# SHI-Labs/Self-Similarity-Grouping

Hardware: AMD Instinct MI355X
Metric: images/s embed + s/iter for NxN rerank+DBSCAN, N=16k, 1/2/4/8 GPU (higher is better)
Workload: dtype f32 (embed: split-half operands hi+lo on fp16 MFMA, fp32 accumulate, 6e-8 max error vs the fp32 reference features) / exact int64 via int8 MFMA digits + f64 + f16 (distance, re-rank: half semantics, bit-exact)

## Files before the change

self-similarity-grouping_amd/csrc/bottleneck.hip:

```cpp
#include "ssg_common.h"
#include <cstdlib>

#ifndef SSG_BN_NT_STORE
#define SSG_BN_NT_STORE 1
#endif
#ifndef SSG_BN_NT_RES
#define SSG_BN_NT_RES 1
#endif

namespace ssg {
namespace bneck {

typedef float v16f __attribute__((ext_vector_type(16)));
typedef unsigned int v4u __attribute__((ext_vector_type(4)));
typedef _Float16 v8h __attribute__((ext_vector_type(8)));
typedef float v4f __attribute__((ext_vector_type(4)));

struct Params {
  const float* x; float* out;
  const float* w1; const float* b1; const float* cs1;
  const float* w2; const float* b2; const float* cs2;
  const float* w3; const float* b3; const float* cs3;
  int B, H;
  int* overflow;
  unsigned long long* prof = nullptr;
};
#ifdef SSG_BN_PROF
#define SSG_BN_STAMP(I_) { if (p.prof && threadIdx.x == 0) p.prof[(size_t)blockIdx.x * 8 + (I_)] = __builtin_readcyclecounter(); }
#else
#define SSG_BN_STAMP(I_)
#endif

constexpr int cmax(int a, int b) { return a > b ? a : b; }

template <int C, int MID, int IW, int TH, int CIN = C, int NW = 4>
struct Cfg {
  static constexpr int HROWS = TH + 2, NPIX1 = HROWS * IW, NPIX = TH * IW;
  static constexpr int NTHR = NW * 64, RPP = NTHR / 4;
#ifndef SSG_BN_K1T
#define SSG_BN_K1T 32
#endif
#ifndef SSG_BN_K1T4
#define SSG_BN_K1T4 32
#endif
  static constexpr int K1T = NW == 8 ? SSG_BN_K1T : SSG_BN_K1T4, KS1 = K1T / 16, CPR1 = 4 * KS1, RPP1 = NTHR / CPR1;
  static constexpr int XROWS = (NPIX1 + RPP1 - 1) / RPP1 * RPP1;
  static constexpr int P1 = 80;
  static constexpr int P1T = K1T * 4 + 16;
  static constexpr int KT2 = NW == 8 ? 2 : 1;
  static constexpr int P2 = KT2 * 128 + 16;
  static constexpr int PY = MID * 4 + 16;
  static constexpr int BUF1 = (XROWS + MID) * P1T;
  static constexpr int ZERO_OFF = NPIX1 * PY;
  static constexpr int W2_OFF = (ZERO_OFF + PY + 255) / 256 * 256, BUF2 = MID * P2;
  static constexpr int W3_OFF = (NPIX * PY + 255) / 256 * 256, BUF3 = C * P1;
  static constexpr int LDS = cmax(cmax(2 * BUF1, W2_OFF + 2 * BUF2), W3_OFF + 2 * BUF3);
  static constexpr int DS = CIN != C;
#ifdef SSG_BN_ABL_NK1
  static constexpr int NK1 = SSG_BN_ABL_NK1;
#else
  static constexpr int NK1 = CIN / K1T;
#endif
  static constexpr int NK2 = (MID / 32) * 9 / KT2, NK3 = (MID + (DS ? CIN : 0)) / 16;
  static constexpr int PD1MAX = K1T == 64 ? 2 : (K1T == 32 ? 4 : 8);
  static constexpr int PD1 = NK1 < PD1MAX ? NK1 : PD1MAX, PD2 = KT2 == 1 ? 6 : 3;
  static_assert(((MID / 32) * 9) % KT2 == 0 && NK2 % PD2 == 0, "phase-2 stages and ring");
  static_assert((NW == 4 || NW == 8) && NPIX == 128 && NPIX1 % 32 == 0 && MID % RPP == 0 && MID % RPP1 == 0 && C % RPP == 0 && MID % (NW * 8) == 0, "128 output pixels, whole staging passes");
  static constexpr bool ZERO_EARLY = 2 * BUF1 <= ZERO_OFF;
  static_assert(LDS <= (NW == 4 ? 80 : 160) * 1024, "4 waves: two workgroups per CU; 8 waves: one");
  static_assert(NW == 4 || NW * 32 * 36 * 4 <= 2 * BUF3, "8 waves: the epilogue patches take over the W3 stages");
};

__device__ __forceinline__ unsigned pack2(_Float16 a, _Float16 b) {
  return (unsigned)__builtin_bit_cast(unsigned short, a) | ((unsigned)__builtin_bit_cast(unsigned short, b) << 16);
}
__device__ __forceinline__ void encode4(const float4 v, uint2& hi, uint2& lo) {
  const _Float16 h0 = (_Float16)v.x, h1 = (_Float16)v.y, h2 = (_Float16)v.z, h3 = (_Float16)v.w;
  hi = make_uint2(pack2(h0, h1), pack2(h2, h3));
  lo = make_uint2(pack2((_Float16)(v.x - (float)h0), (_Float16)(v.y - (float)h1)), pack2((_Float16)(v.z - (float)h2), (_Float16)(v.w - (float)h3)));
}
__device__ __forceinline__ unsigned hi_nonfinite_bits(const uint2 hi) {
  return ((hi.x & 0x7c007c00u) + 0x04000400u) | ((hi.y & 0x7c007c00u) + 0x04000400u);
}
__device__ __forceinline__ float hlo(unsigned u) { return (float)__builtin_bit_cast(_Float16, (unsigned short)(u & 0xffffu)); }
__device__ __forceinline__ float hhi(unsigned u) { return (float)__builtin_bit_cast(_Float16, (unsigned short)(u >> 16)); }
__device__ __forceinline__ float4 decode4(const uint2 hi, const uint2 lo) {
  return make_float4(hlo(hi.x) + hlo(lo.x), hhi(hi.x) + hhi(lo.x), hlo(hi.y) + hlo(lo.y), hhi(hi.y) + hhi(lo.y));
}
__device__ __forceinline__ float4 relu4(float4 v) {
  return make_float4(v.x > 0.f ? v.x : 0.f, v.y > 0.f ? v.y : 0.f, v.z > 0.f ? v.z : 0.f, v.w > 0.f ? v.w : 0.f);
}

__device__ __forceinline__ void bn_dma16(const __amdgpu_buffer_rsrc_t r, unsigned lds_addr, unsigned voff, int soff) {
  __builtin_amdgcn_raw_ptr_buffer_load_lds(r, (__attribute__((address_space(3))) void*)(uintptr_t)lds_addr, 16, voff, soff, 0, 0);
}

template <int C, int MID, int IW, int TH, int CIN, int NW>
__global__ __launch_bounds__(NW * 64, NW == 4 ? 2 : 1) void bottleneck_kernel(Params p) {
  using K = Cfg<C, MID, IW, TH, CIN, NW>;
  constexpr bool DS = K::DS;
  extern __shared__ __attribute__((aligned(16))) unsigned char smem[];
  const int tid = (int)threadIdx.x, lane = tid & 63, wave = tid >> 6, l32 = lane & 31, h = lane >> 5;
  const int tiles_img = p.H / TH, ntiles = p.B * tiles_img;
  int T;
  {
    const int b = (int)blockIdx.x, q = ntiles / 8, r = ntiles % 8, x = b % 8, s = b / 8;
    T = (x < r ? x * (q + 1) : r * (q + 1) + (x - r) * q) + s;
  }
  const int img = T / tiles_img, ty0 = (T - img * tiles_img) * TH;
  SSG_BN_STAMP(0)
  if (K::ZERO_EARLY && tid < K::PY / 16) *reinterpret_cast<uint4*>(smem + K::ZERO_OFF + tid * 16) = make_uint4(0u, 0u, 0u, 0u);

  constexpr int RPP = K::RPP, RPP1 = K::RPP1, AU = K::XROWS / RPP1, WU = MID / RPP1;
  const int ck = tid & 3, r0 = tid >> 2;
  const int ck1 = tid % K::CPR1, r1 = tid / K::CPR1;
  const float* ximg = p.x + (int64_t)img * p.H * IW * CIN;
  const __amdgpu_buffer_rsrc_t xrsrc = __builtin_amdgcn_make_buffer_rsrc(const_cast<float*>(ximg), 0, (unsigned)(p.H * IW * CIN * 4), 0x00020000);
  constexpr int MT1 = K::NPIX1 / 32, NT1 = MID / 32;
  constexpr int WC1 = NT1 < NW / 2 ? NT1 : NW / 2, WR1 = NW / WC1, MTW1 = (MT1 + WR1 - 1) / WR1, NTW1 = NT1 / WC1;
  static_assert(NT1 % WC1 == 0 && (WR1 * MTW1) * 32 <= K::XROWS, "phase-1 tiles divide over the waves");
  const int i1b = (wave / WC1) * MTW1, j1b = (wave % WC1) * NTW1;
  v16f acc1[MTW1][NTW1];
#pragma unroll
  for (int i = 0; i < MTW1; i++)
#pragma unroll
    for (int j = 0; j < NTW1; j++)
#pragma unroll
      for (int r = 0; r < 16; r++) acc1[i][j][r] = 0.f;
  float4 cs1r[NTW1][4], b1r[NTW1][4];
#pragma unroll
  for (int j = 0; j < NTW1; j++)
#pragma unroll
    for (int q = 0; q < 4; q++) {
      cs1r[j][q] = *reinterpret_cast<const float4*>(p.cs1 + (j1b + j) * 32 + 8 * q + 4 * h); b1r[j][q] = *reinterpret_cast<const float4*>(p.b1 + (j1b + j) * 32 + 8 * q + 4 * h);
    }
#ifndef SSG_BN_P1DMA
#define SSG_BN_P1DMA 1
#endif
  if constexpr (NW == 8 && K::K1T == 32 && SSG_BN_P1DMA) {
    constexpr int NS = 4, XR = K::NPIX1, SROWS = XR + MID, STG = SROWS * 128, NBLK = SROWS / 8, TDMA = (NBLK + NW - 1) / NW;
    static_assert(K::NK1 % NS == 0 && NS * STG <= K::LDS && SROWS % 8 == 0 && XR % 8 == 0 && MTW1 == 3 && NTW1 == 1, "phase-1 DMA stages");
    const int wv = __builtin_amdgcn_readfirstlane(wave);
    const __amdgpu_buffer_rsrc_t wrsrc = __builtin_amdgcn_make_buffer_rsrc(const_cast<float*>(p.w1), 0, (unsigned)(MID * CIN * 4), 0x00020000);
    unsigned go[TDMA];
    int gblk[TDMA];
#pragma unroll
    for (int u = 0; u < TDMA; u++) {
      int blk = wv + NW * u;
      if (blk >= NBLK) blk = wv;
      gblk[u] = blk;
      const int r = blk * 8 + (lane >> 3), lc = (lane & 7) ^ ((r >> 1) & 7);
      if (blk < XR / 8) {
        const int pix = (ty0 - 1) * IW + r;
        go[u] = (pix >= 0 && pix < p.H * IW) ? (unsigned)((pix * CIN + lc * 4) * 4) : 0x80000000u;
      } else {
        go[u] = (unsigned)(((r - XR) * CIN + lc * 4) * 4);
      }
    }
#define SSG_BN_DMA1(T_, ST_)                                                                                         \
    { _Pragma("unroll") for (int u = 0; u < TDMA; u++)                                                               \
        bn_dma16(gblk[u] < XR / 8 ? xrsrc : wrsrc, (unsigned)(uintptr_t)(smem + (ST_) * STG + gblk[u] * 1024), go[u], (T_) * 128); }
    const int i1s = __builtin_amdgcn_readfirstlane(i1b);
    int xo[MTW1], xs[MTW1];
#pragma unroll
    for (int i = 0; i < MTW1; i++) { const int r = (i1s + i) * 32 + l32; xo[i] = r * 128; xs[i] = (r >> 1) & 7; }
    const int wr_ = XR + j1b * 32 + l32, wo = wr_ * 128, ws = (wr_ >> 1) & 7;
    v8h fxh[2][2][MTW1], fxl[2][2][MTW1], fwh[2][2], fwl[2][2];
#define SSG_BN_READS1(ST_, S_)                                                                                       \
    { const unsigned char* sb_ = smem + (ST_) * STG;                                                                 \
      _Pragma("unroll") for (int ks = 0; ks < 2; ks++) {                                                             \
        _Pragma("unroll") for (int i = 0; i < MTW1; i++) {                                        \
          fxh[S_][ks][i] = *reinterpret_cast<const v8h*>(sb_ + xo[i] + (((4 * ks + 2 * h) ^ xs[i]) * 16));           \
          fxl[S_][ks][i] = *reinterpret_cast<const v8h*>(sb_ + xo[i] + (((4 * ks + 2 * h + 1) ^ xs[i]) * 16)); }     \
        fwh[S_][ks] = *reinterpret_cast<const v8h*>(sb_ + wo + (((4 * ks + 2 * h) ^ ws) * 16));                       \
        fwl[S_][ks] = *reinterpret_cast<const v8h*>(sb_ + wo + (((4 * ks + 2 * h + 1) ^ ws) * 16)); } }
#define SSG_BN_MMAK(S_, KS_)                                                                                         \
    { _Pragma("unroll") for (int i = 0; i < MTW1; i++) acc1[i][0] = __builtin_amdgcn_mfma_f32_32x32x16_f16(fwh[S_][KS_], fxl[S_][KS_][i], acc1[i][0], 0, 0, 0); \
      _Pragma("unroll") for (int i = 0; i < MTW1; i++) acc1[i][0] = __builtin_amdgcn_mfma_f32_32x32x16_f16(fwl[S_][KS_], fxh[S_][KS_][i], acc1[i][0], 0, 0, 0); \
      _Pragma("unroll") for (int i = 0; i < MTW1; i++) acc1[i][0] = __builtin_amdgcn_mfma_f32_32x32x16_f16(fwh[S_][KS_], fxh[S_][KS_][i], acc1[i][0], 0, 0, 0); }
#define SSG_BN_STEPD(KT_, ST_, STN_, S_)                                                                             \
    { SSG_BN_MMAK(S_, 0)                                                                                             \
      __builtin_amdgcn_sched_barrier(0);                                                                             \
      asm volatile("s_waitcnt vmcnt(%0) lgkmcnt(0)\n\ts_barrier" ::"n"(TDMA * (NS - 2)) : "memory");                  \
      { const int tn_ = (KT_) + NS < K::NK1 ? (KT_) + NS : K::NK1 - 1;    \
        SSG_BN_DMA1(tn_, ST_) }                                                                                      \
      SSG_BN_READS1(STN_, 1 - (S_))                                                                                  \
      __builtin_amdgcn_sched_barrier(0);                                                                             \
      SSG_BN_MMAK(S_, 1) }
    SSG_BN_DMA1(0, 0) SSG_BN_DMA1(1, 1) SSG_BN_DMA1(2, 2) SSG_BN_DMA1(3, 3)
    asm volatile("s_waitcnt vmcnt(%0)\n\ts_barrier" ::"n"(TDMA * (NS - 1)) : "memory");
    SSG_BN_READS1(0, 0)
#pragma unroll 1
    for (int kt = 0; kt < K::NK1; kt += NS) {
      SSG_BN_STEPD(kt, 0, 1, 0) SSG_BN_STEPD(kt + 1, 1, 2, 1) SSG_BN_STEPD(kt + 2, 2, 3, 0) SSG_BN_STEPD(kt + 3, 3, 0, 1)
    }
    __syncthreads();
#undef SSG_BN_STEPD
#undef SSG_BN_MMAK
#undef SSG_BN_READS1
#undef SSG_BN_DMA1
  } else {
  unsigned aoff[AU];
#pragma unroll
  for (int u = 0; u < AU; u++) {
    const int hp = r1 + RPP1 * u, pix = (ty0 - 1) * IW + hp;
    aoff[u] = (hp < K::NPIX1 && pix >= 0 && pix < p.H * IW) ? (unsigned)((pix * CIN + ck1 * 4) * 4) : 0x80000000u;
  }
  const float* w1p = p.w1 + (int64_t)r1 * CIN + ck1 * 4;
  v4f sa[K::PD1][AU], sw[K::PD1][WU];
#define SSG_BN_LOAD1(T_, S_)                                                                                         \
  {                                                                                                                  \
    _Pragma("unroll") for (int u = 0; u < AU; u++) {                                                                  \
      const v4u raw = __builtin_amdgcn_raw_buffer_load_b128(xrsrc, aoff[u], (T_) * (K::K1T * 4), 0);                  \
      sa[S_][u] = __builtin_bit_cast(v4f, raw);                                                                     \
    }                                                                                                                 \
    _Pragma("unroll") for (int u = 0; u < WU; u++) sw[S_][u] = *reinterpret_cast<const v4f*>(w1p + (int64_t)(RPP1 * u) * CIN + (T_) * K::K1T); \
  }
#define SSG_BN_STORE1(BUF_, S_)                                                                                      \
  {                                                                                                                  \
    unsigned char* sb_ = smem + (BUF_) * K::BUF1;                                                                    \
    _Pragma("unroll") for (int u = 0; u < AU; u++) *reinterpret_cast<v4f*>(sb_ + (r1 + RPP1 * u) * K::P1T + ck1 * 16) = sa[S_][u]; \
    _Pragma("unroll") for (int u = 0; u < WU; u++) *reinterpret_cast<v4f*>(sb_ + (K::XROWS + r1 + RPP1 * u) * K::P1T + ck1 * 16) = sw[S_][u]; \
  }
#define SSG_BN_MMA1(BUF_)                                                                                            \
  {                                                                                                                  \
    const unsigned char* sb_ = smem + (BUF_) * K::BUF1;                                                              \
    _Pragma("unroll") for (int ks = 0; ks < K::KS1; ks++) {                                                          \
    v8h xh_[MTW1], xl_[MTW1], wh_[NTW1], wl_[NTW1];                                                                  \
    _Pragma("unroll") for (int i = 0; i < MTW1; i++) {                                                               \
      const unsigned char* q_ = sb_ + ((i1b + i) * 32 + l32) * K::P1T + ks * 64 + h * 32;                            \
      xh_[i] = *reinterpret_cast<const v8h*>(q_); xl_[i] = *reinterpret_cast<const v8h*>(q_ + 16); }                 \
    _Pragma("unroll") for (int j = 0; j < NTW1; j++) {                                                               \
      const unsigned char* q_ = sb_ + (K::XROWS + (j1b + j) * 32 + l32) * K::P1T + ks * 64 + h * 32;                 \
      wh_[j] = *reinterpret_cast<const v8h*>(q_); wl_[j] = *reinterpret_cast<const v8h*>(q_ + 16); }                 \
    _Pragma("unroll") for (int i = 0; i < MTW1; i++) _Pragma("unroll") for (int j = 0; j < NTW1; j++)                \
      acc1[i][j] = __builtin_amdgcn_mfma_f32_32x32x16_f16(wh_[j], xl_[i], acc1[i][j], 0, 0, 0);                      \
    _Pragma("unroll") for (int i = 0; i < MTW1; i++) _Pragma("unroll") for (int j = 0; j < NTW1; j++)                \
      acc1[i][j] = __builtin_amdgcn_mfma_f32_32x32x16_f16(wl_[j], xh_[i], acc1[i][j], 0, 0, 0);                      \
    _Pragma("unroll") for (int i = 0; i < MTW1; i++) _Pragma("unroll") for (int j = 0; j < NTW1; j++)                \
      acc1[i][j] = __builtin_amdgcn_mfma_f32_32x32x16_f16(wh_[j], xh_[i], acc1[i][j], 0, 0, 0);                      \
    }                                                                                                                \
  }
#define SSG_BN_STEP1(KT_, S_)                                                                                        \
  {                                                                                                                  \
    if ((KT_) + K::PD1 < K::NK1) SSG_BN_LOAD1((KT_) + K::PD1, S_)    \
    SSG_BN_MMA1((S_) & 1)                                                                                            \
    if ((KT_) + 1 < K::NK1) SSG_BN_STORE1(((S_) + 1) & 1, ((S_) + 1) % K::PD1)                                        \
    __syncthreads();                                                                                                 \
  }
  static_assert(K::NK1 % K::PD1 == 0 && K::PD1 <= 8, "phase-1 ring of PD1 register sets");
#define SSG_BN_LOAD1_IF(S_) if constexpr ((S_) < K::PD1) SSG_BN_LOAD1(S_, S_)
  SSG_BN_LOAD1_IF(0) SSG_BN_LOAD1_IF(1) SSG_BN_LOAD1_IF(2) SSG_BN_LOAD1_IF(3) SSG_BN_LOAD1_IF(4) SSG_BN_LOAD1_IF(5) SSG_BN_LOAD1_IF(6) SSG_BN_LOAD1_IF(7)
#undef SSG_BN_LOAD1_IF
  SSG_BN_STORE1(0, 0)
  __syncthreads();
#define SSG_BN_STEP1_IF(KT_, S_) if constexpr ((S_) < K::PD1) SSG_BN_STEP1(KT_, S_)
#pragma unroll
  for (int kt0 = 0; kt0 < K::NK1; kt0 += K::PD1) {
    SSG_BN_STEP1_IF(kt0, 0) SSG_BN_STEP1_IF(kt0 + 1, 1) SSG_BN_STEP1_IF(kt0 + 2, 2) SSG_BN_STEP1_IF(kt0 + 3, 3)
    SSG_BN_STEP1_IF(kt0 + 4, 4) SSG_BN_STEP1_IF(kt0 + 5, 5) SSG_BN_STEP1_IF(kt0 + 6, 6) SSG_BN_STEP1_IF(kt0 + 7, 7)
  }
#undef SSG_BN_STEP1_IF
#undef SSG_BN_STEP1
  }
  SSG_BN_STAMP(1)
#undef SSG_BN_LOAD1
#undef SSG_BN_STORE1
#undef SSG_BN_MMA1

  constexpr int CPR2 = 8 * K::KT2, RP8 = K::NTHR / CPR2, BU = MID / RP8;
  const int ck8 = tid % CPR2, r8 = tid / CPR2;
  const float* w2p = p.w2 + (int64_t)r8 * (9 * MID) + ck8 * 4;
  v4f sb2[K::PD2][BU];
#define SSG_BN_LOAD2(T_, S_)                                                                                         \
  { _Pragma("unroll") for (int u = 0; u < BU; u++) sb2[S_][u] = *reinterpret_cast<const v4f*>(w2p + (int64_t)(RP8 * u) * (9 * MID) + (T_) * (32 * K::KT2)); }
#define SSG_BN_STORE2(BUF_, S_)                                                                                      \
  { unsigned char* sb_ = smem + K::W2_OFF + (BUF_) * K::BUF2;                                                        \
    _Pragma("unroll") for (int u = 0; u < BU; u++) *reinterpret_cast<v4f*>(sb_ + (r8 + RP8 * u) * K::P2 + ck8 * 16) = sb2[S_][u]; }
#define SSG_BN_LOAD2_IF(S_) if constexpr ((S_) < K::PD2) SSG_BN_LOAD2(S_, S_)
  SSG_BN_LOAD2_IF(0) SSG_BN_LOAD2_IF(1) SSG_BN_LOAD2_IF(2) SSG_BN_LOAD2_IF(3) SSG_BN_LOAD2_IF(4) SSG_BN_LOAD2_IF(5)
#undef SSG_BN_LOAD2_IF

  unsigned ovf = 0u;
#pragma unroll
  for (int i = 0; i < MTW1; i++) {
    if (i1b + i >= MT1) continue;
    const int hp0 = (i1b + i) * 32;
    const int irow = ty0 - 1 + (hp0 + l32) / IW;
    const bool inside = irow >= 0 && irow < p.H;
#pragma unroll
    for (int j = 0; j < NTW1; j++)
#pragma unroll
      for (int q = 0; q < 4; q++) {
        const int ch = (j1b + j) * 32 + 8 * q + 4 * h;
        const float4 cs = cs1r[j][q], bi = b1r[j][q];
        float4 v = make_float4(acc1[i][j][4 * q] * cs.x + bi.x, acc1[i][j][4 * q + 1] * cs.y + bi.y, acc1[i][j][4 * q + 2] * cs.z + bi.z,
                               acc1[i][j][4 * q + 3] * cs.w + bi.w);
        v = relu4(v);
        if (!inside) v = make_float4(0.f, 0.f, 0.f, 0.f);
        uint2 hi, lo;
        encode4(v, hi, lo);
        ovf |= hi_nonfinite_bits(hi);
        unsigned char* d = smem + (hp0 + l32) * K::PY + (ch >> 3) * 32 + h * 8;
        *reinterpret_cast<uint2*>(d) = hi; *reinterpret_cast<uint2*>(d + 16) = lo;
      }
  }
  if (!K::ZERO_EARLY && tid < K::PY / 16) *reinterpret_cast<uint4*>(smem + K::ZERO_OFF + tid * 16) = make_uint4(0u, 0u, 0u, 0u);
  SSG_BN_STORE2(0, 0)
  __syncthreads();
  SSG_BN_STAMP(2)

  constexpr int WC2 = NW / 4, NT2 = MID / 32 / WC2;
  const int pt2 = wave / WC2, cb2 = (wave % WC2) * NT2;
  v16f acc2[NT2];
#pragma unroll
  for (int j = 0; j < NT2; j++)
#pragma unroll
    for (int r = 0; r < 16; r++) acc2[j][r] = 0.f;
  const int m2 = pt2 * 32 + l32, ty2 = m2 / IW, tx2 = m2 - ty2 * IW;
  float4 cs2r[NT2][4], b2r[NT2][4];
#pragma unroll
  for (int j = 0; j < NT2; j++)
#pragma unroll
    for (int q = 0; q < 4; q++) {
      cs2r[j][q] = *reinterpret_cast<const float4*>(p.cs2 + (cb2 + j) * 32 + 8 * q + 4 * h); b2r[j][q] = *reinterpret_cast<const float4*>(p.b2 + (cb2 + j) * 32 + 8 * q + 4 * h);
    }
#define SSG_BN_STEP2(KT_, S_, B_)                                                                                     \
  {                                                                                                                  \
    if ((KT_) + K::PD2 < K::NK2) SSG_BN_LOAD2((KT_) + K::PD2, S_)                                                     \
    _Pragma("unroll") for (int sub = 0; sub < K::KT2; sub++) {                                                       \
      const int kt_ = (KT_) * K::KT2 + sub;                                                                          \
      const int chunk = kt_ / 9, tap = kt_ - chunk * 9, r = tap / 3, s = tap - r * 3;                                \
      const int xin = tx2 + s - 1;                                                                                   \
      const int abase = (xin >= 0 && xin < IW) ? ((ty2 + r) * IW + xin) * K::PY : K::ZERO_OFF;                       \
      const unsigned char* wb = smem + K::W2_OFF + (B_) * K::BUF2 + (cb2 * 32 + l32) * K::P2 + sub * 128 + h * 32;     \
      v8h xh_[2], xl_[2], wh_[2][NT2], wl_[2][NT2];                                                                  \
      _Pragma("unroll") for (int ks = 0; ks < 2; ks++) {                                                             \
        const unsigned char* q_ = smem + abase + (chunk * 4 + ks * 2 + h) * 32;                                      \
        xh_[ks] = *reinterpret_cast<const v8h*>(q_); xl_[ks] = *reinterpret_cast<const v8h*>(q_ + 16);               \
        _Pragma("unroll") for (int j = 0; j < NT2; j++) {                                                            \
          wh_[ks][j] = *reinterpret_cast<const v8h*>(wb + j * 32 * K::P2 + ks * 64);                                 \
          wl_[ks][j] = *reinterpret_cast<const v8h*>(wb + j * 32 * K::P2 + ks * 64 + 16); }                          \
      }                                                                                                              \
      _Pragma("unroll") for (int ks = 0; ks < 2; ks++) {                                                             \
        _Pragma("unroll") for (int j = 0; j < NT2; j++) acc2[j] = __builtin_amdgcn_mfma_f32_32x32x16_f16(wh_[ks][j], xl_[ks], acc2[j], 0, 0, 0); \
        _Pragma("unroll") for (int j = 0; j < NT2; j++) acc2[j] = __builtin_amdgcn_mfma_f32_32x32x16_f16(wl_[ks][j], xh_[ks], acc2[j], 0, 0, 0); \
        _Pragma("unroll") for (int j = 0; j < NT2; j++) acc2[j] = __builtin_amdgcn_mfma_f32_32x32x16_f16(wh_[ks][j], xh_[ks], acc2[j], 0, 0, 0); \
      }                                                                                                              \
    }                                                                                                                \
    if ((KT_) + 1 < K::NK2) SSG_BN_STORE2((B_) ^ 1, ((S_) + 1) % K::PD2)                                              \
    __syncthreads();                                                                                                 \
  }
  static_assert(K::NK2 % 6 == 0 && 6 % K::PD2 == 0, "phase-2 ring");
#pragma unroll
  for (int kt0 = 0; kt0 < K::NK2; kt0 += 6) {
    SSG_BN_STEP2(kt0, 0 % K::PD2, 0) SSG_BN_STEP2(kt0 + 1, 1 % K::PD2, 1) SSG_BN_STEP2(kt0 + 2, 2 % K::PD2, 0)
    SSG_BN_STEP2(kt0 + 3, 3 % K::PD2, 1) SSG_BN_STEP2(kt0 + 4, 4 % K::PD2, 0) SSG_BN_STEP2(kt0 + 5, 5 % K::PD2, 1)
  }
#undef SSG_BN_STEP2
  SSG_BN_STAMP(3)
#undef SSG_BN_LOAD2
#undef SSG_BN_STORE2

  constexpr int CU3 = C / RPP;
  constexpr int K3 = MID + (DS ? CIN : 0);
  const float* w3p = p.w3 + (int64_t)r0 * K3 + ck * 4;
  v4f sc3[2][CU3];
#define SSG_BN_LOAD3(T_, S_)                                                                                         \
  { _Pragma("unroll") for (int u = 0; u < CU3; u++) sc3[S_][u] = *reinterpret_cast<const v4f*>(w3p + (int64_t)(RPP * u) * K3 + (T_) * 16); }
#define SSG_BN_STORE3(BUF_, S_)                                                                                      \
  { unsigned char* sb_ = smem + K::W3_OFF + (BUF_) * K::BUF3;                                                        \
    _Pragma("unroll") for (int u = 0; u < CU3; u++) *reinterpret_cast<v4f*>(sb_ + (r0 + RPP * u) * K::P1 + ck * 16) = sc3[S_][u]; }
  SSG_BN_LOAD3(0, 0)
  SSG_BN_LOAD3(1, 1)
  constexpr int WC3 = NW / 4, NT3 = C / 32 / WC3;
  const int pt3 = wave / WC3, cb3 = (wave % WC3) * NT3;
  const int64_t gpix0 = ((int64_t)img * p.H + ty0) * IW + pt3 * 32;
  constexpr int NXK = DS ? CIN / 16 : 1;
  v8h xrh[NXK], xrl[NXK];
  if constexpr (DS) {
    const float* xq = p.x + (gpix0 + l32) * CIN + h * 8;
#pragma unroll
    for (int t = 0; t < NXK; t++) { xrh[t] = *reinterpret_cast<const v8h*>(xq + t * 16); xrl[t] = *reinterpret_cast<const v8h*>(xq + t * 16 + 4); }
  }
  unsigned char* myrows = smem + (pt3 * 32) * K::PY;
#pragma unroll
  for (int j = 0; j < NT2; j++)
#pragma unroll
    for (int q = 0; q < 4; q++) {
      const int ch = (cb2 + j) * 32 + 8 * q + 4 * h;
      const float4 cs = cs2r[j][q], bi = b2r[j][q];
      float4 v = make_float4(acc2[j][4 * q] * cs.x + bi.x, acc2[j][4 * q + 1] * cs.y + bi.y, acc2[j][4 * q + 2] * cs.z + bi.z, acc2[j][4 * q + 3] * cs.w + bi.w);
      v = relu4(v);
      uint2 hi, lo;
      encode4(v, hi, lo);
      ovf |= hi_nonfinite_bits(hi);
      unsigned char* d = smem + (pt2 * 32 + l32) * K::PY + (ch >> 3) * 32 + h * 8;
      *reinterpret_cast<uint2*>(d) = hi; *reinterpret_cast<uint2*>(d + 16) = lo;
    }

  static_assert(K::NK3 % 2 == 0, "phase 3 takes its k-tiles in rounds of two buffers");
  v16f acc3[NT3];
#pragma unroll
  for (int j = 0; j < NT3; j++)
#pragma unroll
    for (int r = 0; r < 16; r++) acc3[j][r] = 0.f;
#define SSG_BN_MMA3K(BUF_, KT_)                                                                                      \
  {                                                                                                                  \
    v8h xh_, xl_;                                                                                                    \
    if constexpr (DS && (KT_) >= MID / 16) { xh_ = xrh[((KT_) - MID / 16) % NXK]; xl_ = xrl[((KT_) - MID / 16) % NXK]; } \
    else {                                                                                                           \
      const unsigned char* q_ = myrows + l32 * K::PY + (((KT_) % (MID / 16)) * 2 + h) * 32;                          \
      xh_ = *reinterpret_cast<const v8h*>(q_); xl_ = *reinterpret_cast<const v8h*>(q_ + 16);                         \
    }                                                                                                                \
    const unsigned char* wb_ = smem + K::W3_OFF + (BUF_) * K::BUF3 + (cb3 * 32 + l32) * K::P1 + h * 32;              \
    _Pragma("unroll") for (int jj = 0; jj < NT3; jj += 4) {                                                          \
      v8h wh_[4], wl_[4];                                                                                            \
      _Pragma("unroll") for (int j = 0; j < 4; j++) {                                                                \
        wh_[j] = *reinterpret_cast<const v8h*>(wb_ + (jj + j) * 32 * K::P1); wl_[j] = *reinterpret_cast<const v8h*>(wb_ + (jj + j) * 32 * K::P1 + 16); } \
      _Pragma("unroll") for (int j = 0; j < 4; j++) acc3[jj + j] = __builtin_amdgcn_mfma_f32_32x32x16_f16(wh_[j], xl_, acc3[jj + j], 0, 0, 0); \
      _Pragma("unroll") for (int j = 0; j < 4; j++) acc3[jj + j] = __builtin_amdgcn_mfma_f32_32x32x16_f16(wl_[j], xh_, acc3[jj + j], 0, 0, 0); \
      _Pragma("unroll") for (int j = 0; j < 4; j++) acc3[jj + j] = __builtin_amdgcn_mfma_f32_32x32x16_f16(wh_[j], xh_, acc3[jj + j], 0, 0, 0); \
    }                                                                                                                \
  }
  constexpr int EP = 36, CPR = 8, RPI = 8, ITS = 4;
  const int chunk = lane % CPR, prow = lane / CPR, odd = lane & 1;
  const float* __restrict__ resp = p.x + gpix0 * C;
  float* __restrict__ outp = p.out + gpix0 * C;
  float4 rr[2][ITS], b3r[2], cs3r[2];
#ifdef SSG_BN_ABL_NORES
#define SSG_BN_RESLOAD(P_) make_float4(0.f, 0.f, 0.f, 0.f)
#elif SSG_BN_NT_RES
#define SSG_BN_RESLOAD(P_) ([&]() { const v4f t_ = __builtin_nontemporal_load(reinterpret_cast<const v4f*>(P_)); return make_float4(t_[0], t_[1], t_[2], t_[3]); }())
#else
#define SSG_BN_RESLOAD(P_) (*reinterpret_cast<const float4*>(P_))
#endif
  SSG_BN_STORE3(0, 0)
  SSG_BN_STORE3(1, 1)
  if constexpr (K::NK3 > 2) { SSG_BN_LOAD3(2, 0) SSG_BN_LOAD3(3, 1) }
  __syncthreads();
  static_assert(K::NK3 / 2 <= 4, "at most four rounds");
#define SSG_BN_ROUND3(R_)                                                                                            \
  if constexpr ((R_) < K::NK3 / 2) {                                                                                 \
    SSG_BN_MMA3K(0, 2 * (R_))                                                                                        \
    SSG_BN_MMA3K(1, 2 * (R_) + 1)                                                                                    \
    if constexpr ((R_) + 1 < K::NK3 / 2) {                                                                           \
      __syncthreads();                                                \
      SSG_BN_STORE3(0, 0)                                                                                            \
      SSG_BN_STORE3(1, 1)                                                                                            \
      if constexpr ((R_) + 2 < K::NK3 / 2) { SSG_BN_LOAD3(2 * (R_) + 4, 0) SSG_BN_LOAD3(2 * (R_) + 5, 1) }           \
      else {                                  \
        if constexpr (!DS) {                                                                                         \
          _Pragma("unroll") for (int it = 0; it < ITS; it++) rr[0][it] = SSG_BN_RESLOAD(resp + (int64_t)(it * RPI + prow) * C + cb3 * 32 + chunk * 4); \
        }                                                                                                            \
        b3r[0] = *reinterpret_cast<const float4*>(p.b3 + cb3 * 32 + chunk * 4); cs3r[0] = *reinterpret_cast<const float4*>(p.cs3 + cb3 * 32 + chunk * 4); \
      }                                                                                                              \
      __syncthreads();                                                                                               \
    }                                                                                                                \
  }
  SSG_BN_ROUND3(0) SSG_BN_ROUND3(1) SSG_BN_ROUND3(2) SSG_BN_ROUND3(3)
#undef SSG_BN_ROUND3
  SSG_BN_STAMP(4)
#undef SSG_BN_LOAD3
#undef SSG_BN_STORE3
#undef SSG_BN_MMA3K

  static_assert(32 * EP * 4 <= 32 * K::PY, "patch fits in the wave's y2 rows");
  float* patch;
  if constexpr (WC3 == 1) patch = reinterpret_cast<float*>(myrows);
  else {
    __syncthreads();
    patch = reinterpret_cast<float*>(smem + K::W3_OFF) + wave * (32 * EP);
  }
#pragma unroll
  for (int j = 0; j < NT3; j++) {
    const int col = (cb3 + j) * 32 + chunk * 4;
    if (j + 1 < NT3) {
      if constexpr (!DS) {
#pragma unroll
        for (int it = 0; it < ITS; it++) rr[(j + 1) & 1][it] = SSG_BN_RESLOAD(resp + (int64_t)(it * RPI + prow) * C + col + 32);
      }
      b3r[(j + 1) & 1] = *reinterpret_cast<const float4*>(p.b3 + col + 32); cs3r[(j + 1) & 1] = *reinterpret_cast<const float4*>(p.cs3 + col + 32);
    }
    const float4 bias = b3r[j & 1], cs = cs3r[j & 1];
#pragma unroll
    for (int q = 0; q < 4; q++)
      *reinterpret_cast<float4*>(patch + l32 * EP + 8 * q + 4 * h) = make_float4(acc3[j][4 * q], acc3[j][4 * q + 1], acc3[j][4 * q + 2], acc3[j][4 * q + 3]);
    __builtin_amdgcn_fence(__ATOMIC_ACQ_REL, "wavefront");
#pragma unroll
    for (int it = 0; it < ITS; it++) {
      const int pr = it * RPI + prow;
      float4 v = *reinterpret_cast<const float4*>(patch + pr * EP + chunk * 4);
      v.x = v.x * cs.x + bias.x; v.y = v.y * cs.y + bias.y; v.z = v.z * cs.z + bias.z; v.w = v.w * cs.w + bias.w;
      if constexpr (!DS) {
      const float4 rw = rr[j & 1][it];
      float4 r4;
      {
        const unsigned a0 = __float_as_uint(rw.x), a1 = __float_as_uint(rw.y), a2 = __float_as_uint(rw.z), a3 = __float_as_uint(rw.w);
        const unsigned g0 = lane_xor1((odd ? a0 : a2)), g1 = lane_xor1((odd ? a1 : a3));
        const unsigned h0 = odd ? g0 : a0, h1 = odd ? g1 : a1, l0 = odd ? a2 : g0, l1 = odd ? a3 : g1;
        r4 = decode4(make_uint2(h0, h1), make_uint2(l0, l1));
      }
      v.x += r4.x; v.y += r4.y; v.z += r4.z; v.w += r4.w;
      }
      v = relu4(v);
      uint2 hp, lp;
      encode4(v, hp, lp);
      ovf |= hi_nonfinite_bits(hp);
      const unsigned rx = lane_xor1((odd ? hp.x : lp.x)), ry = lane_xor1((odd ? hp.y : lp.y));
      const uint4 stv = make_uint4(odd ? rx : hp.x, odd ? ry : hp.y, odd ? lp.x : rx, odd ? lp.y : ry);
#if SSG_BN_NT_STORE
      { const v4u sv_ = {stv.x, stv.y, stv.z, stv.w}; __builtin_nontemporal_store(sv_, reinterpret_cast<v4u*>(outp + (int64_t)pr * C + col)); }
#else
      *reinterpret_cast<uint4*>(outp + (int64_t)pr * C + col) = stv;
#endif
    }
    __builtin_amdgcn_fence(__ATOMIC_ACQ_REL, "wavefront");
  }
  if ((ovf & 0x80008000u) && p.overflow) *p.overflow = 1;
  SSG_BN_STAMP(5)
}

}
}

extern "C" int ssg_bottleneck_supported(int H, int W, int CIN, int C, int MID) {
  if (C == 256 && MID == 64 && (CIN == 256 || CIN == 64) && W == 32 && H > 0 && H % 4 == 0) return 1;
  if (C == 512 && MID == 128 && CIN == 512 && W == 16 && H > 0 && H % 8 == 0) return 1;
  return 0;
}

template <int C, int MID, int IW, int TH, int CIN, int NW>
static int launch_bottleneck(const ssg::bneck::Params& p, hipStream_t stream) {
  using namespace ssg::bneck;
  using K = Cfg<C, MID, IW, TH, CIN, NW>;
  static bool attr_set = false;
  if (!attr_set) {
    SSG_HIP(hipFuncSetAttribute((const void*)bottleneck_kernel<C, MID, IW, TH, CIN, NW>, hipFuncAttributeMaxDynamicSharedMemorySize, K::LDS));
    attr_set = true;
  }
  hipLaunchKernelGGL((bottleneck_kernel<C, MID, IW, TH, CIN, NW>), dim3(p.B * (p.H / TH)), dim3(NW * 64), K::LDS, stream, p);
  SSG_LAUNCH_CHECK("bottleneck_kernel");
  return SSG_OK;
}

extern "C" int ssg_bottleneck_nhwc_x(const void* x, const void* w1, const float* b1, const float* cs1, const void* w2, const float* b2, const float* cs2,
                                     const void* w3, const float* b3, const float* cs3, void* out, int B, int H, int W, int C, int MID,
                                     int32_t* overflow, hipStream_t stream) {
  using namespace ssg::bneck;
  if (B <= 0 || !ssg_bottleneck_supported(H, W, C, C, MID) || !cs1 || !cs2 || !cs3 || x == out) {
    ssg_set_error("ssg_bottleneck_nhwc_x: unsupported block B=%d H=%d W=%d C=%d MID=%d (see ssg_bottleneck_supported)", B, H, W, C, MID);
    return SSG_ERR_INVALID;
  }
  Params p;
  p.x = (const float*)x; p.out = (float*)out;
  p.w1 = (const float*)w1; p.b1 = b1; p.cs1 = cs1; p.w2 = (const float*)w2; p.b2 = b2; p.cs2 = cs2; p.w3 = (const float*)w3; p.b3 = b3; p.cs3 = cs3;
  p.B = B; p.H = H; p.overflow = overflow;
  if (C == 512) return launch_bottleneck<512, 128, 16, 8, 512, 8>(p, stream);
  return launch_bottleneck<256, 64, 32, 4, 256, 4>(p, stream);
}

extern "C" int ssg_bottleneck_ds_nhwc_x(const void* x, const void* w1, const float* b1, const float* cs1, const void* w2, const float* b2, const float* cs2,
                                        const void* w3cat, const float* b3, const float* cs3, void* out, int B, int H, int W, int CIN, int C, int MID,
                                        int32_t* overflow, hipStream_t stream) {
  using namespace ssg::bneck;
  if (B <= 0 || CIN == C || !ssg_bottleneck_supported(H, W, CIN, C, MID) || !cs1 || !cs2 || !cs3) {
    ssg_set_error("ssg_bottleneck_ds_nhwc_x: unsupported block B=%d H=%d W=%d CIN=%d C=%d MID=%d (see ssg_bottleneck_supported)", B, H, W, CIN, C, MID);
    return SSG_ERR_INVALID;
  }
  Params p;
  p.x = (const float*)x; p.out = (float*)out;
  p.w1 = (const float*)w1; p.b1 = b1; p.cs1 = cs1; p.w2 = (const float*)w2; p.b2 = b2; p.cs2 = cs2; p.w3 = (const float*)w3cat; p.b3 = b3; p.cs3 = cs3;
  p.B = B; p.H = H; p.overflow = overflow;
  return launch_bottleneck<256, 64, 32, 4, 64, 4>(p, stream);
}
```

Measured before the change: 29160.

## Add 4-wave two-half bottleneck kernel for C=512 layer with two WGs per CU

```diff
diff --git a/self-similarity-grouping_amd/csrc/bottleneck.hip b/self-similarity-grouping_amd/csrc/bottleneck.hip
--- a/self-similarity-grouping_amd/csrc/bottleneck.hip
+++ b/self-similarity-grouping_amd/csrc/bottleneck.hip
@@ -521,6 +521,331 @@
   SSG_BN_STAMP(5)
 }
 
+template <int C, int MID, int IW, int TH>
+struct CfgH {
+  static constexpr int NW = 4, NTHR = NW * 64, HROWS = TH + 2, NPIX1 = HROWS * IW, NPIX = TH * IW;
+  static constexpr int MH = MID / 2;
+  static constexpr int K1T = 32, P1T = K1T * 4, CPR1 = 8, RPP1 = NTHR / CPR1;
+  static constexpr int XROWS = NPIX1, BUF1 = (XROWS + MID) * P1T;
+  static constexpr int NK1 = C / K1T, PD1 = 2;
+  static constexpr int PYH = MH * 4 + 16;
+  static constexpr int ZERO_OFF = NPIX1 * PYH;
+  static constexpr int P2 = 144, W2_OFF = (ZERO_OFF + PYH + 255) / 256 * 256, BUF2 = MID * P2;
+  static constexpr int NK2H = (MH / 32) * 9, PD2 = 3;
+  static constexpr int NCP = 128, NPASS = C / NCP, KT3 = MID / 32;
+  static constexpr int EP = 36, PATCH = 32 * EP * 4;
+  static constexpr int LDS = cmax(2 * BUF1, W2_OFF + 2 * BUF2);
+  static_assert(NPIX == 128 && NPIX1 % RPP1 == 0 && MID % RPP1 == 0 && MH == 64 && MID == NCP && NK1 % PD1 == 0 && NK2H % 6 == 0 && KT3 == 4, "layer2 shape");
+  static_assert(((NPIX1 + 31) / 32 + 1) / 2 == 3 && 6 * 32 <= XROWS + MID, "phase 1: 2 x 3 pixel tiles, the sixth one reads W1 rows of the stage");
+  static_assert(RPP1 % 16 == 0 && XROWS % 16 == 0, "the swizzle of a row is that of its thread (r1) / its lane (l32)");
+  static_assert(NW * PATCH <= ZERO_OFF && 32 * P2 == PATCH, "patches live in the dead y1 rows");
+  static_assert(LDS <= 80 * 1024, "two workgroups per CU");
+};
+
+template <int C, int MID, int IW, int TH>
+__global__ __launch_bounds__(256, 2) void bottleneck_halves_kernel(Params p) {
+  using K = CfgH<C, MID, IW, TH>;
+  extern __shared__ __attribute__((aligned(16))) unsigned char smem[];
+  const int tid = (int)threadIdx.x, lane = tid & 63, wave = tid >> 6, l32 = lane & 31, h = lane >> 5;
+  const int tiles_img = p.H / TH, ntiles = p.B * tiles_img;
+  int T;
+  {
+    const int b = (int)blockIdx.x, q = ntiles / 8, r = ntiles % 8, x = b % 8, s = b / 8;
+    T = (x < r ? x * (q + 1) : r * (q + 1) + (x - r) * q) + s;
+  }
+  const int img = T / tiles_img, ty0 = (T - img * tiles_img) * TH;
+  SSG_BN_STAMP(0)
+
+  constexpr int RPP1 = K::RPP1, AU = K::XROWS / RPP1, WU = MID / RPP1, MT1 = K::NPIX1 / 32, MTW1 = 3;
+  const int ck1 = tid & 7, r1 = tid >> 3;
+  const float* ximg = p.x + (int64_t)img * p.H * IW * C;
+  const __amdgpu_buffer_rsrc_t xrsrc = __builtin_amdgcn_make_buffer_rsrc(const_cast<float*>(ximg), 0, (unsigned)(p.H * IW * C * 4), 0x00020000);
+  const int i1b = (wave >> 1) * MTW1, j1b = wave & 1;
+  v16f acc1[MTW1][2];
+#pragma unroll
+  for (int i = 0; i < MTW1; i++)
+#pragma unroll
+    for (int j = 0; j < 2; j++)
+#pragma unroll
+      for (int r = 0; r < 16; r++) acc1[i][j][r] = 0.f;
+  {
+    unsigned aoff[AU];
+#pragma unroll
+    for (int u = 0; u < AU; u++) {
+      const int pix = (ty0 - 1) * IW + r1 + RPP1 * u;
+      aoff[u] = (pix >= 0 && pix < p.H * IW) ? (unsigned)((pix * C + ck1 * 4) * 4) : 0x80000000u;
+    }
+    const float* w1p = p.w1 + (int64_t)r1 * C + ck1 * 4;
+    const int wsw = ((ck1 ^ ((r1 >> 1) & 7)) * 16), rsw = (l32 >> 1) & 7;
+    v4f sa[K::PD1][AU], sw[K::PD1][WU];
+#define SSG_BH_LOAD1(T_, S_)                                                                                         \
+    {                                                                                                                \
+      _Pragma("unroll") for (int u = 0; u < AU; u++) {                                                                \
+        const v4u raw = __builtin_amdgcn_raw_buffer_load_b128(xrsrc, aoff[u], (T_) * (K::K1T * 4), 0);                \
+        sa[S_][u] = __builtin_bit_cast(v4f, raw);                                                                   \
+      }                                                                                                               \
+      _Pragma("unroll") for (int u = 0; u < WU; u++) sw[S_][u] = *reinterpret_cast<const v4f*>(w1p + (int64_t)(RPP1 * u) * C + (T_) * K::K1T); \
+    }
+#define SSG_BH_STORE1(BUF_, S_)                                                                                      \
+    {                                                                                                                \
+      unsigned char* sb_ = smem + (BUF_) * K::BUF1;                                                                  \
+      _Pragma("unroll") for (int u = 0; u < AU; u++) *reinterpret_cast<v4f*>(sb_ + (r1 + RPP1 * u) * K::P1T + wsw) = sa[S_][u]; \
+      _Pragma("unroll") for (int u = 0; u < WU; u++) *reinterpret_cast<v4f*>(sb_ + (K::XROWS + r1 + RPP1 * u) * K::P1T + wsw) = sw[S_][u]; \
+    }
+#define SSG_BH_MMA1(BUF_)                                                                                            \
+    {                                                                                                                \
+      const unsigned char* sb_ = smem + (BUF_) * K::BUF1;                                                            \
+      _Pragma("unroll") for (int ks = 0; ks < 2; ks++) {                                                             \
+        const int ch_ = ((4 * ks + 2 * h) ^ rsw) * 16, cl_ = ((4 * ks + 2 * h + 1) ^ rsw) * 16;                      \
+        v8h xh_[MTW1], xl_[MTW1], wh_[2], wl_[2];                                                                    \
+        _Pragma("unroll") for (int i = 0; i < MTW1; i++) {                                                           \
+          const unsigned char* q_ = sb_ + ((i1b + i) * 32 + l32) * K::P1T;                                           \
+          xh_[i] = *reinterpret_cast<const v8h*>(q_ + ch_); xl_[i] = *reinterpret_cast<const v8h*>(q_ + cl_); }      \
+        _Pragma("unroll") for (int j = 0; j < 2; j++) {                                                              \
+          const unsigned char* q_ = sb_ + (K::XROWS + (j1b + 2 * j) * 32 + l32) * K::P1T;                            \
+          wh_[j] = *reinterpret_cast<const v8h*>(q_ + ch_); wl_[j] = *reinterpret_cast<const v8h*>(q_ + cl_); }      \
+        _Pragma("unroll") for (int i = 0; i < MTW1; i++) _Pragma("unroll") for (int j = 0; j < 2; j++)               \
+          acc1[i][j] = __builtin_amdgcn_mfma_f32_32x32x16_f16(wh_[j], xl_[i], acc1[i][j], 0, 0, 0);                  \
+        _Pragma("unroll") for (int i = 0; i < MTW1; i++) _Pragma("unroll") for (int j = 0; j < 2; j++)               \
+          acc1[i][j] = __builtin_amdgcn_mfma_f32_32x32x16_f16(wl_[j], xh_[i], acc1[i][j], 0, 0, 0);                  \
+        _Pragma("unroll") for (int i = 0; i < MTW1; i++) _Pragma("unroll") for (int j = 0; j < 2; j++)               \
+          acc1[i][j] = __builtin_amdgcn_mfma_f32_32x32x16_f16(wh_[j], xh_[i], acc1[i][j], 0, 0, 0);                  \
+      }                                                                                                              \
+    }
+#define SSG_BH_STEP1(KT_, S_)                                                                                        \
+    {                                                                                                                \
+      if ((KT_) + K::PD1 < K::NK1) SSG_BH_LOAD1((KT_) + K::PD1, S_)                                                   \
+      SSG_BH_MMA1(S_)                                                                                                \
+      if ((KT_) + 1 < K::NK1) SSG_BH_STORE1(1 - (S_), 1 - (S_))                                                       \
+      __syncthreads();                                                                                               \
+    }
+    SSG_BH_LOAD1(0, 0) SSG_BH_LOAD1(1, 1)
+    SSG_BH_STORE1(0, 0)
+    __syncthreads();
+#pragma unroll 1
+    for (int kt0 = 0; kt0 < K::NK1; kt0 += 2) { SSG_BH_STEP1(kt0, 0) SSG_BH_STEP1(kt0 + 1, 1) }
+#undef SSG_BH_STEP1
+#undef SSG_BH_MMA1
+#undef SSG_BH_STORE1
+#undef SSG_BH_LOAD1
+  }
+  SSG_BN_STAMP(1)
+
+  constexpr int RP8 = K::NTHR / 8, BU = MID / RP8;
+  const int ck8 = tid & 7, r8 = tid >> 3;
+  const float* w2p = p.w2 + (int64_t)r8 * (9 * MID) + ck8 * 4;
+  const int m2 = wave * 32 + l32, ty2 = m2 / IW, tx2 = m2 - ty2 * IW;
+  constexpr int NT2 = MID / 32;
+  v16f acc2[NT2];
+#pragma unroll
+  for (int j = 0; j < NT2; j++)
+#pragma unroll
+    for (int r = 0; r < 16; r++) acc2[j][r] = 0.f;
+  unsigned ovf = 0u;
+  v4f sb2[K::PD2][BU];
+#define SSG_BH_LOAD2(T_, S_)                                                                                         \
+  { _Pragma("unroll") for (int u = 0; u < BU; u++) sb2[S_][u] = *reinterpret_cast<const v4f*>(w2p + (int64_t)(RP8 * u) * (9 * MID) + (T_) * 32); }
+#define SSG_BH_STORE2(BUF_, S_)                                                                                      \
+  { unsigned char* sb_ = smem + K::W2_OFF + (BUF_) * K::BUF2;                                                        \
+    _Pragma("unroll") for (int u = 0; u < BU; u++) *reinterpret_cast<v4f*>(sb_ + (r8 + RP8 * u) * K::P2 + ck8 * 16) = sb2[S_][u]; }
+#define SSG_BH_STEP2(HF_, KT_, S_, B_)                                                                                \
+  {                                                                                                                  \
+    if ((KT_) + K::PD2 < K::NK2H) SSG_BH_LOAD2((HF_) * K::NK2H + (KT_) + K::PD2, S_)                                  \
+    {                                                                                                                \
+      const int cl = (KT_) / 9, tap = (KT_) - cl * 9, r = tap / 3, s = tap - r * 3;    \
+      const int xin = tx2 + s - 1;                                                                                   \
+      const int abase = (xin >= 0 && xin < IW) ? ((ty2 + r) * IW + xin) * K::PYH : K::ZERO_OFF;                      \
+      const unsigned char* wb = smem + K::W2_OFF + (B_) * K::BUF2 + l32 * K::P2 + h * 32;                             \
+      _Pragma("unroll") for (int ks = 0; ks < 2; ks++) {                                                             \
+        const unsigned char* q_ = smem + abase + (cl * 4 + ks * 2 + h) * 32;                                         \
+        const v8h xh_ = *reinterpret_cast<const v8h*>(q_), xl_ = *reinterpret_cast<const v8h*>(q_ + 16);             \
+        v8h wh_[NT2], wl_[NT2];                                                                                      \
+        _Pragma("unroll") for (int j = 0; j < NT2; j++) {                                                            \
+          wh_[j] = *reinterpret_cast<const v8h*>(wb + j * 32 * K::P2 + ks * 64);                                     \
+          wl_[j] = *reinterpret_cast<const v8h*>(wb + j * 32 * K::P2 + ks * 64 + 16); }                              \
+        _Pragma("unroll") for (int j = 0; j < NT2; j++) acc2[j] = __builtin_amdgcn_mfma_f32_32x32x16_f16(wh_[j], xl_, acc2[j], 0, 0, 0); \
+        _Pragma("unroll") for (int j = 0; j < NT2; j++) acc2[j] = __builtin_amdgcn_mfma_f32_32x32x16_f16(wl_[j], xh_, acc2[j], 0, 0, 0); \
+        _Pragma("unroll") for (int j = 0; j < NT2; j++) acc2[j] = __builtin_amdgcn_mfma_f32_32x32x16_f16(wh_[j], xh_, acc2[j], 0, 0, 0); \
+      }                                                                                                              \
+    }                                                                                                                \
+    if ((KT_) + 1 < K::NK2H) SSG_BH_STORE2((B_) ^ 1, ((S_) + 1) % K::PD2)                                             \
+    __syncthreads();                                                                                                 \
+  }
+#define SSG_BH_HALF(HF_)                                                                                             \
+  {                                                                                                                  \
+    SSG_BH_LOAD2((HF_) * K::NK2H, 0) SSG_BH_LOAD2((HF_) * K::NK2H + 1, 1) SSG_BH_LOAD2((HF_) * K::NK2H + 2, 2)        \
+    float4 cs1r[4], b1r[4];                                                                                          \
+    _Pragma("unroll") for (int q = 0; q < 4; q++) {                                                                  \
+      cs1r[q] = *reinterpret_cast<const float4*>(p.cs1 + (HF_) * K::MH + j1b * 32 + 8 * q + 4 * h);                  \
+      b1r[q] = *reinterpret_cast<const float4*>(p.b1 + (HF_) * K::MH + j1b * 32 + 8 * q + 4 * h); }                  \
+    _Pragma("unroll") for (int i = 0; i < MTW1; i++) {                                                               \
+      if (i1b + i >= MT1) continue;                                  \
+      const int hp0 = (i1b + i) * 32;                                        \
+      const int irow = ty0 - 1 + (hp0 + l32) / IW;                                                                   \
+      const bool inside = irow >= 0 && irow < p.H;                                                                   \
+      _Pragma("unroll") for (int q = 0; q < 4; q++) {                                                                \
+        const int ch = j1b * 32 + 8 * q + 4 * h;                                        \
+        const float4 cs = cs1r[q], bi = b1r[q];                                                                      \
+        float4 v = make_float4(acc1[i][HF_][4 * q] * cs.x + bi.x, acc1[i][HF_][4 * q + 1] * cs.y + bi.y, acc1[i][HF_][4 * q + 2] * cs.z + bi.z, \
+                               acc1[i][HF_][4 * q + 3] * cs.w + bi.w);                                               \
+        v = relu4(v);                                                                                                \
+        if (!inside) v = make_float4(0.f, 0.f, 0.f, 0.f);                                                            \
+        uint2 hi, lo;                                                                                                \
+        encode4(v, hi, lo);                                                                                          \
+        ovf |= hi_nonfinite_bits(hi);                                                                                \
+        unsigned char* d = smem + (hp0 + l32) * K::PYH + (ch >> 3) * 32 + h * 8;                                     \
+        *reinterpret_cast<uint2*>(d) = hi; *reinterpret_cast<uint2*>(d + 16) = lo;                                   \
+      }                                                                                                              \
+    }                                                                                                                \
+    if ((HF_) == 0 && tid < K::PYH / 16) *reinterpret_cast<uint4*>(smem + K::ZERO_OFF + tid * 16) = make_uint4(0u, 0u, 0u, 0u);    \
+    SSG_BH_STORE2(0, 0)                                                                                              \
+    __syncthreads();                                                                                                 \
+    _Pragma("unroll 1") for (int kt0 = 0; kt0 < K::NK2H; kt0 += 6) {                                                 \
+      SSG_BH_STEP2(HF_, kt0, 0, 0) SSG_BH_STEP2(HF_, kt0 + 1, 1, 1) SSG_BH_STEP2(HF_, kt0 + 2, 2, 0)                  \
+      SSG_BH_STEP2(HF_, kt0 + 3, 0, 1) SSG_BH_STEP2(HF_, kt0 + 4, 1, 0) SSG_BH_STEP2(HF_, kt0 + 5, 2, 1)              \
+    }                                                                                                                \
+    SSG_BN_STAMP(2 + (HF_))                                                                                          \
+  }
+  SSG_BH_HALF(0)
+  SSG_BH_HALF(1)
+#undef SSG_BH_HALF
+#undef SSG_BH_STEP2
+#undef SSG_BH_STORE2
+#undef SSG_BH_LOAD2
+
+  constexpr int NS3 = K::NPASS * K::KT3;
+  const float* w3p = p.w3 + (int64_t)r8 * MID + ck8 * 4;
+  v4f sc3[2][BU];
+#define SSG_BH_LOAD3(T_, S_)                                                                                         \
+  { _Pragma("unroll") for (int u = 0; u < BU; u++)                                                                    \
+      sc3[S_][u] = *reinterpret_cast<const v4f*>(w3p + (int64_t)(((T_) / K::KT3) * K::NCP + RP8 * u) * MID + ((T_) % K::KT3) * 32); }
+#define SSG_BH_STORE3(BUF_, S_)                                                                                      \
+  { unsigned char* sb_ = smem + K::W2_OFF + (BUF_) * K::BUF2;                                                        \
+    _Pragma("unroll") for (int u = 0; u < BU; u++) *reinterpret_cast<v4f*>(sb_ + (r8 + RP8 * u) * K::P2 + ck8 * 16) = sc3[S_][u]; }
+  SSG_BH_LOAD3(0, 0)
+  SSG_BH_LOAD3(1, 1)
+
+  unsigned char* const patchb = smem + wave * K::PATCH;
+  v8h y2h[MID / 16], y2l[MID / 16];
+#pragma unroll
+  for (int j = 0; j < NT2; j++) {
+#pragma unroll
+    for (int q = 0; q < 4; q++) {
+      const float4 cs = *reinterpret_cast<const float4*>(p.cs2 + j * 32 + 8 * q + 4 * h), bi = *reinterpret_cast<const float4*>(p.b2 + j * 32 + 8 * q + 4 * h);
+      float4 v = make_float4(acc2[j][4 * q] * cs.x + bi.x, acc2[j][4 * q + 1] * cs.y + bi.y, acc2[j][4 * q + 2] * cs.z + bi.z, acc2[j][4 * q + 3] * cs.w + bi.w);
+      v = relu4(v);
+      uint2 hi, lo;
+      encode4(v, hi, lo);
+      ovf |= hi_nonfinite_bits(hi);
+      unsigned char* d = patchb + l32 * K::P2 + q * 32 + h * 8;
+      *reinterpret_cast<uint2*>(d) = hi; *reinterpret_cast<uint2*>(d + 16) = lo;
+    }
+    __builtin_amdgcn_fence(__ATOMIC_ACQ_REL, "wavefront");
+#pragma unroll
+    for (int ks = 0; ks < 2; ks++) {
+      const unsigned char* q_ = patchb + l32 * K::P2 + (ks * 2 + h) * 32;
+      y2h[j * 2 + ks] = *reinterpret_cast<const v8h*>(q_); y2l[j * 2 + ks] = *reinterpret_cast<const v8h*>(q_ + 16);
+    }
+    __builtin_amdgcn_fence(__ATOMIC_ACQ_REL, "wavefront");
+  }
+  SSG_BH_STORE3(0, 0)
+  __syncthreads();
+  SSG_BN_STAMP(4)
+
+  constexpr int EP = K::EP, CPR = 8, RPI = 8, ITS = 4, NT3 = K::NCP / 32;
+  const int chunk = lane % CPR, prow = lane / CPR, odd = lane & 1;
+  const int64_t gpix0 = ((int64_t)img * p.H + ty0) * IW + wave * 32;
+  const float* __restrict__ resp = p.x + gpix0 * C;
+  float* __restrict__ outp = p.out + gpix0 * C;
+  float* const patch = reinterpret_cast<float*>(patchb);
+#if SSG_BN_NT_RES
+#define SSG_BH_RESLOAD(P_) ([&]() { const v4f t_ = __builtin_nontemporal_load(reinterpret_cast<const v4f*>(P_)); return make_float4(t_[0], t_[1], t_[2], t_[3]); }())
+#else
+#define SSG_BH_RESLOAD(P_) (*reinterpret_cast<const float4*>(P_))
+#endif
+#pragma unroll 1
+  for (int ps = 0; ps < K::NPASS; ps++) {
+    const int cb3 = ps * NT3;
+    v16f acc3[NT3];
+#pragma unroll
+    for (int j = 0; j < NT3; j++)
+#pragma unroll
+      for (int r = 0; r < 16; r++) acc3[j][r] = 0.f;
+    float4 rr[2][ITS], b3r[2], cs3r[2];
+#define SSG_BH_STEP3(I_)                                                                                             \
+    {                                                                                                                \
+      const int s_ = ps * K::KT3 + (I_);                                                                             \
+      if (s_ + 2 < NS3) SSG_BH_LOAD3(s_ + 2, (I_) & 1)                                                                \
+      if constexpr ((I_) == K::KT3 - 1) {     \
+        _Pragma("unroll") for (int it = 0; it < ITS; it++) rr[0][it] = SSG_BH_RESLOAD(resp + (int64_t)(it * RPI + prow) * C + cb3 * 32 + chunk * 4); \
+        b3r[0] = *reinterpret_cast<const float4*>(p.b3 + cb3 * 32 + chunk * 4); cs3r[0] = *reinterpret_cast<const float4*>(p.cs3 + cb3 * 32 + chunk * 4); \
+      }                                                                                                              \
+      const unsigned char* wb_ = smem + K::W2_OFF + ((I_) & 1) * K::BUF2 + l32 * K::P2 + h * 32;                      \
+      _Pragma("unroll") for (int ks = 0; ks < 2; ks++) {                                                             \
+        const v8h xh_ = y2h[(I_) * 2 + ks], xl_ = y2l[(I_) * 2 + ks];                                                \
+        v8h wh_[NT3], wl_[NT3];                                                                                      \
+        _Pragma("unroll") for (int j = 0; j < NT3; j++) {                                                            \
+          wh_[j] = *reinterpret_cast<const v8h*>(wb_ + j * 32 * K::P2 + ks * 64);                                    \
+          wl_[j] = *reinterpret_cast<const v8h*>(wb_ + j * 32 * K::P2 + ks * 64 + 16); }                             \
+        _Pragma("unroll") for (int j = 0; j < NT3; j++) acc3[j] = __builtin_amdgcn_mfma_f32_32x32x16_f16(wh_[j], xl_, acc3[j], 0, 0, 0); \
+        _Pragma("unroll") for (int j = 0; j < NT3; j++) acc3[j] = __builtin_amdgcn_mfma_f32_32x32x16_f16(wl_[j], xh_, acc3[j], 0, 0, 0); \
+        _Pragma("unroll") for (int j = 0; j < NT3; j++) acc3[j] = __builtin_amdgcn_mfma_f32_32x32x16_f16(wh_[j], xh_, acc3[j], 0, 0, 0); \
+      }                                                                                                              \
+      if (s_ + 1 < NS3) SSG_BH_STORE3(((I_) + 1) & 1, ((I_) + 1) & 1)                                                 \
+      __syncthreads();                                                                                               \
+    }
+    SSG_BH_STEP3(0) SSG_BH_STEP3(1) SSG_BH_STEP3(2) SSG_BH_STEP3(3)
+#undef SSG_BH_STEP3
+
+#pragma unroll
+    for (int j = 0; j < NT3; j++) {
+      const int col = (cb3 + j) * 32 + chunk * 4;
+      if (j + 1 < NT3) {
+#pragma unroll
+        for (int it = 0; it < ITS; it++) rr[(j + 1) & 1][it] = SSG_BH_RESLOAD(resp + (int64_t)(it * RPI + prow) * C + col + 32);
+        b3r[(j + 1) & 1] = *reinterpret_cast<const float4*>(p.b3 + col + 32); cs3r[(j + 1) & 1] = *reinterpret_cast<const float4*>(p.cs3 + col + 32);
+      }
+      const float4 bias = b3r[j & 1], cs = cs3r[j & 1];
+#pragma unroll
+      for (int q = 0; q < 4; q++)
+        *reinterpret_cast<float4*>(patch + l32 * EP + 8 * q + 4 * h) = make_float4(acc3[j][4 * q], acc3[j][4 * q + 1], acc3[j][4 * q + 2], acc3[j][4 * q + 3]);
+      __builtin_amdgcn_fence(__ATOMIC_ACQ_REL, "wavefront");
+#pragma unroll
+      for (int it = 0; it < ITS; it++) {
+        const int pr = it * RPI + prow;
+        float4 v = *reinterpret_cast<const float4*>(patch + pr * EP + chunk * 4);
+        v.x = v.x * cs.x + bias.x; v.y = v.y * cs.y + bias.y; v.z = v.z * cs.z + bias.z; v.w = v.w * cs.w + bias.w;
+        const float4 rw = rr[j & 1][it];
+        float4 r4;
+        {
+          const unsigned a0 = __float_as_uint(rw.x), a1 = __float_as_uint(rw.y), a2 = __float_as_uint(rw.z), a3 = __float_as_uint(rw.w);
+          const unsigned g0 = lane_xor1((odd ? a0 : a2)), g1 = lane_xor1((odd ? a1 : a3));
+          const unsigned h0 = odd ? g0 : a0, h1 = odd ? g1 : a1, l0 = odd ? a2 : g0, l1 = odd ? a3 : g1;
+          r4 = decode4(make_uint2(h0, h1), make_uint2(l0, l1));
+        }
+        v.x += r4.x; v.y += r4.y; v.z += r4.z; v.w += r4.w;
+        v = relu4(v);
+        uint2 hp, lp;
+        encode4(v, hp, lp);
+        ovf |= hi_nonfinite_bits(hp);
+        const unsigned rx = lane_xor1((odd ? hp.x : lp.x)), ry = lane_xor1((odd ? hp.y : lp.y));
+        const uint4 stv = make_uint4(odd ? rx : hp.x, odd ? ry : hp.y, odd ? lp.x : rx, odd ? lp.y : ry);
+#if SSG_BN_NT_STORE
+        { const v4u sv_ = {stv.x, stv.y, stv.z, stv.w}; __builtin_nontemporal_store(sv_, reinterpret_cast<v4u*>(outp + (int64_t)pr * C + col)); }
+#else
+        *reinterpret_cast<uint4*>(outp + (int64_t)pr * C + col) = stv;
+#endif
+      }
+      __builtin_amdgcn_fence(__ATOMIC_ACQ_REL, "wavefront");
+    }
+  }
+#undef SSG_BH_RESLOAD
+#undef SSG_BH_STORE3
+#undef SSG_BH_LOAD3
+  if ((ovf & 0x80008000u) && p.overflow) *p.overflow = 1;
+  SSG_BN_STAMP(5)
+}
+
 }
 }
 
@@ -544,6 +869,24 @@
   return SSG_OK;
 }
 
+template <int C, int MID, int IW, int TH>
+static int launch_bottleneck_halves(const ssg::bneck::Params& p, hipStream_t stream) {
+  using namespace ssg::bneck;
+  using K = CfgH<C, MID, IW, TH>;
+  static bool attr_set = false;
+  if (!attr_set) {
+    SSG_HIP(hipFuncSetAttribute((const void*)bottleneck_halves_kernel<C, MID, IW, TH>, hipFuncAttributeMaxDynamicSharedMemorySize, K::LDS));
+    attr_set = true;
+  }
+  hipLaunchKernelGGL((bottleneck_halves_kernel<C, MID, IW, TH>), dim3(p.B * (p.H / TH)), dim3(K::NTHR), K::LDS, stream, p);
+  SSG_LAUNCH_CHECK("bottleneck_halves_kernel");
+  return SSG_OK;
+}
+
+#ifndef SSG_BN_L2_WAVES_DEFAULT
+#define SSG_BN_L2_WAVES_DEFAULT 4
+#endif
+
 extern "C" int ssg_bottleneck_nhwc_x(const void* x, const void* w1, const float* b1, const float* cs1, const void* w2, const float* b2, const float* cs2,
                                      const void* w3, const float* b3, const float* cs3, void* out, int B, int H, int W, int C, int MID,
                                      int32_t* overflow, hipStream_t stream) {
@@ -556,7 +899,14 @@
   p.x = (const float*)x; p.out = (float*)out;
   p.w1 = (const float*)w1; p.b1 = b1; p.cs1 = cs1; p.w2 = (const float*)w2; p.b2 = b2; p.cs2 = cs2; p.w3 = (const float*)w3; p.b3 = b3; p.cs3 = cs3;
   p.B = B; p.H = H; p.overflow = overflow;
-  if (C == 512) return launch_bottleneck<512, 128, 16, 8, 512, 8>(p, stream);
+  if (C == 512) {
+    const char* e = getenv("SSG_BN_L2_WAVES");
+    const int nw = e && *e ? atoi(e) : SSG_BN_L2_WAVES_DEFAULT;
+    if (nw == 4) return launch_bottleneck_halves<512, 128, 16, 8>(p, stream);
+    if (nw == 8) return launch_bottleneck<512, 128, 16, 8, 512, 8>(p, stream);
+    ssg_set_error("ssg_bottleneck_nhwc_x: SSG_BN_L2_WAVES=%s (4 or 8)", e);
+    return SSG_ERR_INVALID;
+  }
   return launch_bottleneck<256, 64, 32, 4, 256, 4>(p, stream);
 }
 
```

After: 29520 (median of 6 runs). 1.2% higher.
